# CESSProject/DeOSS

Hardware: AMD Instinct MI355X
Metric: device-resident GiB/s hashed to Merkle root; 1/2/4/8 MI355X scaling (higher is better)
Workload: dtype u32; 1 GPU; BASELINE configs[1]: 1 object of 8 GiB (8589934592 B) in 1 chunk-range shard(s) of 8 GiB, chunk 33554432 B (256 leaves); object_bytes=8589934592, chunk=33554432, leaves=256, parallelism=single GPU

## Files before the change

deoss_amd/csrc/merkle_kernels.hpp:

```cpp
#pragma once
#include "quad_ring.hpp"
#include "sha256_gfx950.hpp"

namespace dm {

constexpr int kBlock = 256;
constexpr int kLeafFuseMax = 8;
constexpr int kReduceTile = 512;

struct LeafArgs {
    const uint8_t* base;
    uint64_t pitch;
    uint64_t leaf_len;
    uint64_t last_len;
    const uint64_t* addrs;
    const uint64_t* lens;
    uint64_t nleaves;
    uint64_t byte_off;
    uint64_t byte_end;
    uint32_t* state;
    uint8_t* digests;
    uint8_t* level_out;
    uint32_t fuse_levels;
};
// ... 345 lines not shown
#pragma unroll
        for (int k = 0; k < 8; k++) o8[k] = res[threadIdx.x][k];
        const uint64_t o = (uint64_t)blockIdx.x * (kLatLeaves >> a.fuse_levels) + threadIdx.x;
        store_digest(a.level_out + 32 * o, o8);
    }
}

constexpr int kPairLeaves = 32;
constexpr int kPairFuseMax = 5;

__device__ __forceinline__ uint32_t dpp_swap_pairs(uint32_t v) {
    return (uint32_t)__builtin_amdgcn_update_dpp(0, (int)v, 0xB1, 0xF, 0xF, true);
}

#define DM_PAIR_ROUND(X4, X5, X6, X7, kw)                                              \
    do {                                                                               \
        const uint32_t s_ = xor3(__builtin_amdgcn_alignbit(X4, X4, sh1),               \
                                 __builtin_amdgcn_alignbit(X4, X4, sh2),               \
                                 __builtin_amdgcn_alignbit(X4, X4, sh3));              \
        const uint32_t x_ = __builtin_amdgcn_bitop3_b32(X4, X5, msk, 0x1e);            \
        const uint32_t f_ = __builtin_amdgcn_bitop3_b32(x_, X6, X5, 0xca);             \
        const uint32_t t_ = s_ + f_ + ((X7 & msk) + (kw));                             \
        const uint32_t y_ = lane_b ? X7 : t_;                                          \
        X7 = t_ + dpp_swap_pairs(y_);                                                  \
    } while (0)

__device__ __forceinline__ void pair_rounds_from_kw(uint32_t (&x)[4], const uint4 (*kw)[kLatLeaves], uint32_t lane,
                                                    uint32_t sh1, uint32_t sh2, uint32_t sh3, uint32_t msk,
                                                    bool lane_b) {
    uint32_t x4 = x[0], x5 = x[1], x6 = x[2], x7 = x[3];
    uint4 q = kw[0][lane];
#pragma unroll
    for (int g = 0; g < 16; g++) {
        uint4 nq = q;
        if (g + 1 < 16) nq = kw[g + 1][lane];
        DM_PAIR_ROUND(x4, x5, x6, x7, q.x);
        DM_PAIR_ROUND(x7, x4, x5, x6, q.y);
        DM_PAIR_ROUND(x6, x7, x4, x5, q.z);
        DM_PAIR_ROUND(x5, x6, x7, x4, q.w);
        q = nq;
    }
    x[0] += x4; x[1] += x5; x[2] += x6; x[3] += x7;
}

template <bool TABLE, bool ALIGNED>
__global__ __launch_bounds__(kLatThreads) void leaf_kernel_pair(LeafArgs a) {
    __shared__ uint4 ring[kLatRing][16][kLatLeaves];
    __shared__ uint32_t lds_a[kPairLeaves][8];
    __shared__ uint32_t lds_b[kPairLeaves / 2][8];
    const uint32_t lane = threadIdx.x & (kLatLeaves - 1);
    const bool producer = __builtin_amdgcn_readfirstlane(threadIdx.x) < kLatLeaves;
    const bool lane_b = (lane & 1) != 0;
    const uint32_t c = lane >> 1;
    const uint64_t first = (uint64_t)blockIdx.x * kPairLeaves;
    const uint64_t i = first + c;
    const LeafView v = leaf_view<TABLE>(a, i);
    const uint64_t NB = wave_max_u64(v.nb);
    if (producer) {
        Blk cur;
        if (v.nb > 0 && !lane_b) cur = load_block<ALIGNED>(v.p);
        for (uint64_t b = 0; b < NB; b++) {
            if (b < v.nb) {
                uint32_t w[16];
                block_words(cur, w);
                if (b + 1 < v.nb && !lane_b) cur = load_block<ALIGNED>(v.p + 64 * (b + 1));
                uint4 (*kw)[kLatLeaves] = ring[b % kLatRing];
#pragma unroll
                for (int q = 0; q < 16; q++) {
                    uint32_t u[4];
#pragma unroll
                    for (int j = 0; j < 4; j++) {
                        const int t = 4 * q + j;
                        uint32_t wt;
                        if (t < 16) {
                            wt = w[t];
                        } else {
                            wt = ssig1(w[(t - 2) & 15]) + w[(t - 7) & 15] + ssig0(w[(t - 15) & 15]) + w[t & 15];
                            w[t & 15] = wt;
                        }
                        u[j] = lane_b ? 0u : kSha256K[t] + wt;
                    }
                    kw[q][lane] = make_uint4(u[0], u[1], u[2], u[3]);
                }
            }
            __syncthreads();
        }
        __syncthreads();
    } else {
        const uint32_t sh1 = lane_b ? 2 : 6, sh2 = lane_b ? 13 : 11, sh3 = lane_b ? 22 : 25;
        const uint32_t msk = lane_b ? 0u : ~0u;
        uint32_t st0[8];
        if (v.active) load_or_init_state(a, i, st0);
        else init_state(st0);
        uint32_t x[4];
#pragma unroll
        for (int k = 0; k < 4; k++) x[k] = lane_b ? st0[k] : st0[4 + k];
        __syncthreads();
        for (uint64_t b = 0; b < NB; b++) {
            if (b < v.nb) pair_rounds_from_kw(x, ring[b % kLatRing], lane, sh1, sh2, sh3, msk, lane_b);
            __syncthreads();
        }
        uint32_t st[8];
#pragma unroll
        for (int k = 0; k < 4; k++) {
            const uint32_t other = dpp_swap_pairs(x[k]);
            st[k] = lane_b ? x[k] : other;
            st[4 + k] = lane_b ? other : x[k];
        }
        if (v.active && !lane_b) {
            leaf_epilogue<ALIGNED>(a, i, v, st);
#pragma unroll
            for (int k = 0; k < 8; k++) lds_a[c][k] = st[k];
        }
    }
    if (a.fuse_levels == 0) return;
    __syncthreads();
    const uint32_t cnt = (uint32_t)((a.nleaves - first) < kPairLeaves ? (a.nleaves - first) : kPairLeaves);
    uint32_t (*res)[8];
    const uint32_t out_cnt = lds_reduce(lds_a, lds_b, cnt, a.fuse_levels, &res);
    if (threadIdx.x < out_cnt) {
        uint32_t o8[8];
#pragma unroll
        for (int k = 0; k < 8; k++) o8[k] = res[threadIdx.x][k];
        const uint64_t o = (uint64_t)blockIdx.x * (kPairLeaves >> a.fuse_levels) + threadIdx.x;
        store_digest(a.level_out + 32 * o, o8);
    }
}

constexpr int kQuadLeaves = 8;
constexpr int kQuadBlocks = 8;
constexpr int kQuadFuseMax = 3;
constexpr int kQuadRow = kQuadLeaves;
constexpr size_t kQuadLdsBytes = sizeof(uint4) * kLatRing * 16 * kQuadBlocks * kQuadRow + 4 * 8 * kQuadLeaves +
                                 4 * 8 * (kQuadLeaves / 2);
static_assert(4 * kQuadLdsBytes <= (160u << 10), "four compact K1Q workgroups must fit a CU's LDS");

#define DM_QS_HEAD(X4, X5, X6)                                                                   \
    "v_alignbit_b32 %[r], %[" X4 "], %[" X4 "], %[sh]\n\t"                                      \
    "v_bitop3_b32 %[f], %[" X4 "], %[" X5 "], %[msk] bitop3:0x1e\n\t"                          \
    "v_bitop3_b32 %[f], %[f], %[" X6 "], %[" X5 "] bitop3:0xca\n\t"                             \
    "v_xor_b32_dpp %[s], %[r], %[r] quad_perm:[1,2,0,3] row_mask:0xf bank_mask:0xf\n\t"
#define DM_QS_SIGMA "v_xor_b32_dpp %[s], %[r], %[s] quad_perm:[2,0,1,3] row_mask:0xf bank_mask:0xf\n\t"
#define DM_QS_STEP_Q(X4, X5, X6, X7, H, HN, VN, QP)                                             \
    DM_QS_HEAD(X4, X5, X6)                                                                       \
    "v_sub_u32_dpp %[" X6 "], %[" VN "], %[" X6 "] quad_perm:" QP " row_mask:0xf bank_mask:0x3\n\t" \
    DM_QS_SIGMA                                                                                  \
    "v_sub_u32_dpp %[" HN "], %[" X4 "], %[" X6 "] row_ror:8 row_mask:0xf bank_mask:0xf\n\t"    \
    "v_add3_u32 %[" X7 "], %[s], %[f], %[" H "]\n\t"
#define DM_QS_STEP(X4, X5, X6, X7, H, HN, VN) DM_QS_STEP_Q(X4, X5, X6, X7, H, HN, VN, "[0,1,2,3]")
#define DM_QS_STEP_A(X4, X5, X6, X7, H, HN)                                                     \
    DM_QS_HEAD(X4, X5, X6)                                                                       \
    DM_QS_SIGMA                                                                                  \
    "v_sub_u32_dpp %[" HN "], %[" X4 "], %[" X6 "] row_ror:8 row_mask:0xf bank_mask:0xf\n\t"    \
    "v_add3_u32 %[" X7 "], %[s], %[f], %[" H "]\n\t"
#define DM_QS_STEP_END(X4, X5, X6, X7, H)                                                       \
    DM_QS_HEAD(X4, X5, X6)                                                                       \
    DM_QS_SIGMA                                                                                  \
    "v_add3_u32 %[" X7 "], %[s], %[f], %[" H "]\n\t"
#define DM_QS_STEPS4V(V0, V1, V2, V3)                                                          \
    DM_QS_STEP("a", "b", "c", "d", "h", "g", V0) DM_QS_STEP("d", "a", "b", "c", "g", "h", V1)   \
    DM_QS_STEP("c", "d", "a", "b", "h", "g", V2) DM_QS_STEP("b", "c", "d", "a", "g", "h", V3)
#define DM_QS_ALIGN_MIS ".p2align 3\n\t.if %[mis]\n\ts_nop 0\n\t.endif\n\t"
#define DM_QS_PROLOGUE(V) DM_QS_PROLOGUE_AT(V, DM_QS_ALIGN_MIS, "[0,1,2,3]")
#define DM_QS_PROLOGUE_AT(V, ALIGN, QP)                                                           \
    "s_nop 1\n\t" ALIGN                                                                          \
    "v_sub_u32_dpp %[d], %[" V "], %[d] quad_perm:" QP " row_mask:0xf bank_mask:0x3\n\t"         \
    "v_sub_u32_dpp %[h], %[b], %[d] row_ror:8 row_mask:0xf bank_mask:0xf\n\t"
#define DM_QS_RESTORE_A(P, X) "v_mov_b32_dpp %[" P "], %[" X "] quad_perm:[0,1,2,3] row_mask:0xf bank_mask:0xc\n\t"
#define DM_QS_GROUP0(V0, V1, V2, V3)                                                             \
    DM_QS_STEP("a", "b", "c", "d", "h", "g", V0) DM_QS_RESTORE_A("d", "x3")                      \
    DM_QS_STEP("d", "a", "b", "c", "g", "h", V1) DM_QS_RESTORE_A("c", "x2")                      \
    DM_QS_STEP("c", "d", "a", "b", "h", "g", V2) DM_QS_STEP("b", "c", "d", "a", "g", "h", V3)
#define DM_QS_FF(X, P, BANKS) "v_add_u32_dpp %[" X "], %[" P "], %[" X "] quad_perm:[0,1,2,3] row_mask:0xf bank_mask:" BANKS "\n\t"
#define DM_QS_TAIL(V0, V1, V2)                                                                   \
    DM_QS_STEP("a", "b", "c", "d", "h", "g", V0) DM_QS_STEP("d", "a", "b", "c", "g", "h", V1)   \
    DM_QS_STEP("c", "d", "a", "b", "h", "g", V2) DM_QS_STEP_A("b", "c", "d", "a", "g", "h")      \
    DM_QS_FF("x3", "d", "0x3") DM_QS_FF("x2", "c", "0x3") DM_QS_FF("x1", "b", "0x3")             \
    DM_QS_FF("x0", "a", "0x3")                                                                   \
    DM_QS_STEP_A("a", "b", "c", "d", "h", "g") DM_QS_STEP_END("d", "a", "b", "c", "g")           \
    DM_QS_FF("x0", "a", "0xc") DM_QS_FF("x1", "b", "0xc") DM_QS_FF("x3", "d", "0xc")             \
    DM_QS_FF("x2", "c", "0xc")
#define DM_QS_STEPS4Q(V0, Q0, V1, Q1, V2, Q2, V3, Q3)                                          \
    DM_QS_STEP_Q("a", "b", "c", "d", "h", "g", V0, Q0) DM_QS_STEP_Q("d", "a", "b", "c", "g", "h", V1, Q1) \
    DM_QS_STEP_Q("c", "d", "a", "b", "h", "g", V2, Q2) DM_QS_STEP_Q("b", "c", "d", "a", "g", "h", V3, Q3)
#define DM_QS_GROUP0Q(V0, Q0, V1, Q1, V2, Q2, V3, Q3)                                          \
    DM_QS_STEP_Q("a", "b", "c", "d", "h", "g", V0, Q0) DM_QS_RESTORE_A("d", "x3")              \
    DM_QS_STEP_Q("d", "a", "b", "c", "g", "h", V1, Q1) DM_QS_RESTORE_A("c", "x2")              \
    DM_QS_STEP_Q("c", "d", "a", "b", "h", "g", V2, Q2) DM_QS_STEP_Q("b", "c", "d", "a", "g", "h", V3, Q3)
#define DM_QS_TAILQ(V0, Q0, V1, Q1, V2, Q2)                                                     \
    DM_QS_STEP_Q("a", "b", "c", "d", "h", "g", V0, Q0) DM_QS_STEP_Q("d", "a", "b", "c", "g", "h", V1, Q1) \
    DM_QS_STEP_Q("c", "d", "a", "b", "h", "g", V2, Q2) DM_QS_STEP_A("b", "c", "d", "a", "g", "h") \
    DM_QS_FF("x3", "d", "0x3") DM_QS_FF("x2", "c", "0x3") DM_QS_FF("x1", "b", "0x3")             \
    DM_QS_FF("x0", "a", "0x3")                                                                   \
    DM_QS_STEP_A("a", "b", "c", "d", "h", "g") DM_QS_STEP_END("d", "a", "b", "c", "g")           \
    DM_QS_FF("x0", "a", "0xc") DM_QS_FF("x1", "b", "0xc") DM_QS_FF("x3", "d", "0xc")             \
    DM_QS_FF("x2", "c", "0xc")
#define DM_QS_OUT                                                                                \
    : [a] "+v"(p0), [b] "+v"(p1), [c] "+v"(p2), [d] "+v"(p3), [h] "+v"(h), [g] "+v"(g),           \
      [x0] "+v"(x[0]), [x1] "+v"(x[1]), [x2] "+v"(x[2]), [x3] "+v"(x[3]), [r] "=&v"(r_),          \
      [f] "=&v"(f_), [s] "=&v"(s_)
#define DM_QS_OPS DM_QS_OUT : [mis] "i"(MIS ? 1 : 0), [sh] "v"(sh.x), [msk] "v"(msk), [v0] "v"(v0), [v1] "v"(v1), [v2] "v"(v2), [v3] "v"(v3)

template <bool MIS, class KW>
__device__ __forceinline__ void quad_block_skewed(uint32_t (&x)[4], KW kw, uint3 sh, uint32_t msk) {
    uint32_t p0 = x[0], p1 = x[1], p2 = x[2], p3 = x[3], h = 0, g = 0, r_, f_, s_;
    uint4 q = kw(0), nq = kw(1);
    {
        const uint32_t v0 = q.x, v1 = 0, v2 = 0, v3 = 0;
        asm volatile(DM_QS_PROLOGUE("v0") DM_QS_OPS);
    }
#pragma unroll
    for (int grp = 0; grp < 16; grp++) {
        const uint4 nnq = grp + 2 < 16 ? kw(grp + 2) : nq;
        const uint32_t v0 = q.y, v1 = q.z, v2 = q.w, v3 = nq.x;
        if (grp == 0) {
            asm volatile(DM_QS_ALIGN_MIS DM_QS_GROUP0("v0", "v1", "v2", "v3") DM_QS_OPS);
        } else if (grp < 15) {
            asm volatile(DM_QS_ALIGN_MIS DM_QS_STEPS4V("v0", "v1", "v2", "v3") DM_QS_OPS);
        } else {
            asm volatile(DM_QS_ALIGN_MIS DM_QS_TAIL("v0", "v1", "v2") DM_QS_OPS);
        }
        q = nq;
        nq = nnq;
    }
}

constexpr int kLgkmWait0 = 0xC07F;

#define DM_QS_HNB(HN, A, B, BANKS) "v_sub_u32_dpp %[" HN "], %[" A "], %[" B "] row_ror:8 row_mask:0xf bank_mask:" BANKS "\n\t"
#define DM_QS_ADDB(D, A, B, BANKS) "v_add_u32_dpp %[" D "], %[" A "], %[" B "] quad_perm:[0,1,2,3] row_mask:0xf bank_mask:" BANKS "\n\t"
#define DM_QS_MOVB(D, S, BANKS) "v_mov_b32_dpp %[" D "], %[" S "] quad_perm:[0,1,2,3] row_mask:0xf bank_mask:" BANKS "\n\t"
#define DM_QS_KWN(X6, S, N) "v_sub_u32_dpp %[" X6 "], %[" N "], %[" S "] quad_perm:[0,0,0,0] row_mask:0xf bank_mask:0x3\n\t"
#define DM_QS_ADD3(X7, H) "v_add3_u32 %[" X7 "], %[s], %[f], %[" H "]\n\t"
#define DM_QS_LINKQ(V0, Q0, V1, Q1, V2, Q2, N0, N1, N2)                                          \
    DM_QS_STEP_Q("a", "b", "c", "d", "h", "g", V0, Q0) DM_QS_STEP_Q("d", "a", "b", "c", "g", "h", V1, Q1) \
    DM_QS_STEP_Q("c", "d", "a", "b", "h", "g", V2, Q2)                                           \
    DM_QS_ADDB("x1", "x1", "b", "0xc") DM_QS_ADDB("x3", "x3", "d", "0x3")                        \
                                            \
    DM_QS_HEAD("b", "c", "d") DM_QS_KWN("d", "x3", N0) DM_QS_SIGMA                               \
    DM_QS_HNB("h", "x1", "d", "0x3") DM_QS_HNB("h", "b", "d", "0xc") DM_QS_ADD3("a", "g")        \
    DM_QS_ADDB("b", "x1", "b", "0x3") DM_QS_ADDB("c", "x2", "c", "0x3")                          \
    DM_QS_HNB("g", "a", "c", "0xc") DM_QS_ADDB("x0", "x0", "a", "0xc")                           \
    DM_QS_ADDB("a", "a", "x0", "0x3") DM_QS_MOVB("x2", "c", "0x3")                               \
                                                            \
    DM_QS_HEAD("a", "b", "c") DM_QS_KWN("c", "c", N1) DM_QS_SIGMA                                \
    DM_QS_HNB("g", "x0", "c", "0x3") DM_QS_ADD3("d", "h")                                        \
    DM_QS_ADDB("x3", "x3", "d", "0xc") DM_QS_MOVB("x1", "b", "0x3") DM_QS_MOVB("x0", "a", "0x3") \
                                           \
    DM_QS_HEAD("d", "a", "b") DM_QS_KWN("b", "b", N2) DM_QS_SIGMA                                \
    DM_QS_HNB("h", "x3", "b", "0x3") DM_QS_HNB("h", "d", "x1", "0xc") DM_QS_ADD3("c", "g")       \
    DM_QS_ADDB("x2", "x2", "c", "0xc") DM_QS_MOVB("a", "x0", "0xc") DM_QS_MOVB("d", "x3", "0xc") \
    DM_QS_MOVB("c", "x2", "0xc")
#define DM_QS_BODYQ                                                                              \
    DM_QS_STEPS4Q("q01", "[1,1,1,1]", "q02", "[1,1,1,1]", "q03", "[1,1,1,1]", "q00", "[2,2,2,2]") \
    DM_QS_STEPS4Q("q01", "[2,2,2,2]", "q02", "[2,2,2,2]", "q03", "[2,2,2,2]", "q00", "[3,3,3,3]") \
    DM_QS_STEPS4Q("q01", "[3,3,3,3]", "q02", "[3,3,3,3]", "q03", "[3,3,3,3]", "q10", "[0,0,0,0]") \
    DM_QS_STEPS4Q("q11", "[0,0,0,0]", "q12", "[0,0,0,0]", "q13", "[0,0,0,0]", "q10", "[1,1,1,1]") \
    DM_QS_STEPS4Q("q11", "[1,1,1,1]", "q12", "[1,1,1,1]", "q13", "[1,1,1,1]", "q10", "[2,2,2,2]") \
    DM_QS_STEPS4Q("q11", "[2,2,2,2]", "q12", "[2,2,2,2]", "q13", "[2,2,2,2]", "q10", "[3,3,3,3]") \
    DM_QS_STEPS4Q("q11", "[3,3,3,3]", "q12", "[3,3,3,3]", "q13", "[3,3,3,3]", "q20", "[0,0,0,0]") \
    DM_QS_STEPS4Q("q21", "[0,0,0,0]", "q22", "[0,0,0,0]", "q23", "[0,0,0,0]", "q20", "[1,1,1,1]") \
    DM_QS_STEPS4Q("q21", "[1,1,1,1]", "q22", "[1,1,1,1]", "q23", "[1,1,1,1]", "q20", "[2,2,2,2]") \
    DM_QS_STEPS4Q("q21", "[2,2,2,2]", "q22", "[2,2,2,2]", "q23", "[2,2,2,2]", "q20", "[3,3,3,3]") \
    DM_QS_STEPS4Q("q21", "[3,3,3,3]", "q22", "[3,3,3,3]", "q23", "[3,3,3,3]", "q30", "[0,0,0,0]") \
    DM_QS_STEPS4Q("q31", "[0,0,0,0]", "q32", "[0,0,0,0]", "q33", "[0,0,0,0]", "q30", "[1,1,1,1]") \
    DM_QS_STEPS4Q("q31", "[1,1,1,1]", "q32", "[1,1,1,1]", "q33", "[1,1,1,1]", "q30", "[2,2,2,2]") \
    DM_QS_STEPS4Q("q31", "[2,2,2,2]", "q32", "[2,2,2,2]", "q33", "[2,2,2,2]", "q30", "[3,3,3,3]")
#define DM_QS_FILLQ                                                                              \
    DM_QS_PROLOGUE_AT("q00", DM_QS_ALIGN_MIS, "[0,0,0,0]")                                       \
    DM_QS_GROUP0Q("q01", "[0,0,0,0]", "q02", "[0,0,0,0]", "q03", "[0,0,0,0]", "q00", "[1,1,1,1]")
#define DM_QS_CONTQ                                                                              \
    DM_QS_ALIGN_MIS                                                                              \
    DM_QS_STEP_Q("c", "d", "a", "b", "h", "g", "q03", "[0,0,0,0]") DM_QS_STEP_Q("b", "c", "d", "a", "g", "h", "q00", "[1,1,1,1]")
#define DM_QS_ENDLINKQ DM_QS_LINKQ("q31", "[3,3,3,3]", "q32", "[3,3,3,3]", "q33", "[3,3,3,3]", "n0", "n1", "n2")
#define DM_QS_ENDTAILQ DM_QS_TAILQ("q31", "[3,3,3,3]", "q32", "[3,3,3,3]", "q33", "[3,3,3,3]")
#define DM_QS_STATE [a] "+v"(P[0]), [b] "+v"(P[1]), [c] "+v"(P[2]), [d] "+v"(P[3]),              \
                    [x0] "+v"(x[0]), [x1] "+v"(x[1]), [x2] "+v"(x[2]), [x3] "+v"(x[3]),           \
                    [r] "=&v"(r_), [f] "=&v"(f_), [s] "=&v"(s_)
#define DM_QS_KIN [mis] "i"(MIS ? 1 : 0), [sh] "v"(sh.x), [msk] "v"(msk),                        \
                  [q00] "v"(K[0].x), [q01] "v"(K[0].y), [q02] "v"(K[0].z), [q03] "v"(K[0].w),     \
                  [q10] "v"(K[1].x), [q11] "v"(K[1].y), [q12] "v"(K[1].z), [q13] "v"(K[1].w),     \
                  [q20] "v"(K[2].x), [q21] "v"(K[2].y), [q22] "v"(K[2].z), [q23] "v"(K[2].w),     \
                  [q30] "v"(K[3].x), [q31] "v"(K[3].y), [q32] "v"(K[3].z), [q33] "v"(K[3].w)

template <bool MIS, int K8>
__device__ __forceinline__ void quad_block_regs(uint32_t (&x)[4], uint32_t (&P)[4], uint32_t& h, uint32_t& g,
                                                const uint4 (&K)[4], const uint4& N, uint3 sh, uint32_t msk) {
    uint32_t r_, f_, s_;
    if constexpr (K8 == 0) {
        asm volatile(DM_QS_FILLQ DM_QS_BODYQ DM_QS_ENDLINKQ
                     : DM_QS_STATE, [h] "=&v"(h), [g] "=&v"(g)
                     : DM_QS_KIN, [n0] "v"(N.x), [n1] "v"(N.y), [n2] "v"(N.z));
    } else if constexpr (K8 < kQuadBlocks - 1) {
        asm volatile(DM_QS_CONTQ DM_QS_BODYQ DM_QS_ENDLINKQ
                     : DM_QS_STATE, [h] "+v"(h), [g] "+v"(g)
                     : DM_QS_KIN, [n0] "v"(N.x), [n1] "v"(N.y), [n2] "v"(N.z));
    } else {
        asm volatile(DM_QS_CONTQ DM_QS_BODYQ DM_QS_ENDTAILQ
                     : DM_QS_STATE, [h] "+v"(h), [g] "+v"(g)
                     : DM_QS_KIN);
    }
}

template <int G, int ROW, bool MIS, int K8 = 0>
__device__ __forceinline__ void quad_stage_blocks(uint32_t (&x)[4], uint32_t (&P)[4], uint32_t& h, uint32_t& g,
                                                  uint4 (&S)[3][4], const uint4* kw, uint3 sh, uint32_t msk) {
    __builtin_amdgcn_s_waitcnt(kLgkmWait0);
    if constexpr (K8 + 2 < kQuadBlocks) {
#pragma unroll
        for (int t = 0; t < 4; t++) S[(K8 + 2) % 3][t] = kw[(K8 + 2) * ROW + 4 * t * G];
    }
    quad_block_regs<MIS, K8>(x, P, h, g, S[K8 % 3], S[(K8 + 1) % 3][0], sh, msk);
    if constexpr (K8 + 1 < kQuadBlocks) quad_stage_blocks<G, ROW, MIS, K8 + 1>(x, P, h, g, S, kw, sh, msk);
}
template <int G, int ROW, bool MIS>
__device__ __forceinline__ void quad_stage_regs(uint32_t (&x)[4], const uint4* kw, uint3 sh, uint32_t msk) {
    uint4 S[3][4];
    uint32_t P[4] = {x[0], x[1], x[2], x[3]}, h, g;
#pragma unroll
    for (int k = 0; k < 2; k++) {
#pragma unroll
        for (int t = 0; t < 4; t++) S[k][t] = kw[k * ROW + 4 * t * G];
    }
    quad_stage_blocks<G, ROW, MIS>(x, P, h, g, S, kw, sh, msk);
}

constexpr int kQuadWideRing = quad_ring::kWideDepth;
constexpr int kQuadSets = quad_ring::kSets;
template <int G, int ROW, int K8, bool FILL, bool TAIL, bool LOAD>
__device__ __forceinline__ void quad_xstage_block(uint32_t (&x)[4], uint32_t (&P)[4], uint32_t& h, uint32_t& g,
                                                  uint4 (&S)[kQuadSets][4], const uint4* src, uint3 sh, uint32_t msk) {
    static_assert((LOAD || !quad_ring::block_prefetches(K8, true)) && (!TAIL || !quad_ring::block_links(K8, true)) &&
                      !(FILL && TAIL) && quad_ring::prefetch_of(K8).block == (K8 + quad_ring::kAhead) % kQuadBlocks,
                  "only the last stage of a run skips a load or drains: quad_ring.hpp");
    __builtin_amdgcn_s_waitcnt(kLgkmWait0);
    if constexpr (LOAD) {
        constexpr quad_ring::BlockRef pf = quad_ring::prefetch_of(K8);
#pragma unroll
        for (int t = 0; t < 4; t++) S[quad_ring::set_of(K8 + quad_ring::kAhead)][t] = src[pf.block * ROW + 4 * t * G];
    }
    quad_block_regs<false, FILL ? 0 : TAIL ? kQuadBlocks - 1 : 1>(x, P, h, g, S[quad_ring::set_of(K8)],
                                                                 S[quad_ring::set_of(K8 + 1)][0], sh, msk);
}
template <int G, int ROW>
__device__ __forceinline__ uint32_t quad_run_xstage(uint32_t (&x)[4], const uint4* colp, uint32_t slot, uint64_t n,
                                                    uint3 sh, uint32_t msk) {
    uint4 S[kQuadSets][4];
    uint32_t P[4] = {x[0], x[1], x[2], x[3]}, h, g;
    const uint4* cur = colp + slot * 16 * G;
#pragma unroll
    for (int k = 0; k < quad_ring::kAhead; k++) {
#pragma unroll
        for (int t = 0; t < 4; t++) S[k][t] = cur[k * ROW + 4 * t * G];
    }
    quad_xstage_block<G, ROW, 0, true, false, true>(x, P, h, g, S, cur, sh, msk);
    for (uint64_t s = 1; s < n; s++) {
        slot = quad_ring::next_slot(slot, kQuadWideRing);
        const uint4* nxt = colp + slot * 16 * G;
        quad_xstage_block<G, ROW, 1, false, false, true>(x, P, h, g, S, cur, sh, msk);
        quad_xstage_block<G, ROW, 2, false, false, true>(x, P, h, g, S, cur, sh, msk);
        quad_xstage_block<G, ROW, 3, false, false, true>(x, P, h, g, S, cur, sh, msk);
        quad_xstage_block<G, ROW, 4, false, false, true>(x, P, h, g, S, cur, sh, msk);
        quad_xstage_block<G, ROW, 5, false, false, true>(x, P, h, g, S, cur, sh, msk);
        quad_xstage_block<G, ROW, 6, false, false, true>(x, P, h, g, S, nxt, sh, msk);
        quad_xstage_block<G, ROW, 7, false, false, true>(x, P, h, g, S, nxt, sh, msk);
        __syncthreads();
        quad_xstage_block<G, ROW, 0, false, false, true>(x, P, h, g, S, nxt, sh, msk);
        cur = nxt;
    }
    quad_xstage_block<G, ROW, 1, false, false, true>(x, P, h, g, S, cur, sh, msk);
    quad_xstage_block<G, ROW, 2, false, false, true>(x, P, h, g, S, cur, sh, msk);
    quad_xstage_block<G, ROW, 3, false, false, true>(x, P, h, g, S, cur, sh, msk);
    quad_xstage_block<G, ROW, 4, false, false, true>(x, P, h, g, S, cur, sh, msk);
    quad_xstage_block<G, ROW, 5, false, false, true>(x, P, h, g, S, cur, sh, msk);
    quad_xstage_block<G, ROW, 6, false, false, false>(x, P, h, g, S, cur, sh, msk);
    quad_xstage_block<G, ROW, 7, false, true, false>(x, P, h, g, S, cur, sh, msk);
    __syncthreads();
    return quad_ring::next_slot(slot, kQuadWideRing);
}

template <bool ALIGNED, int G>
__device__ __forceinline__ void quad_produce_block(const LeafView& v, Blk& cur, uint64_t b, uint4* kw) {
    if (b >= v.nb) return;
    uint32_t w[16];
    block_words(cur, w);
    if (b + kQuadBlocks < v.nb) cur = load_block<ALIGNED>(v.p + 64 * (b + kQuadBlocks));
#pragma unroll
    for (int q = 0; q < 16; q++) {
        uint32_t u[4];
#pragma unroll
        for (int k = 0; k < 4; k++) {
            const int t = 4 * q + k;
            uint32_t wt;
            if (t < 16) {
                wt = w[t];
            } else {
                wt = ssig1(w[(t - 2) & 15]) + w[(t - 7) & 15] + ssig0(w[(t - 15) & 15]) + w[t & 15];
                w[t & 15] = wt;
            }
            u[k] = 0u - (kSha256K[t] + wt);
        }
        kw[q * G] = make_uint4(u[0], u[1], u[2], u[3]);
    }
}

template <bool TABLE, bool ALIGNED, bool COMPACT>
__global__ __launch_bounds__(kLatThreads) void leaf_kernel_quad(LeafArgs a) {
    constexpr int ROW = COMPACT ? kQuadRow : kQuadLeaves;
    constexpr int G = kQuadBlocks * ROW;
    constexpr int DEPTH = COMPACT ? kLatRing : kQuadWideRing;
    __shared__ uint4 ring[COMPACT ? 1 : 2][kLatRing][16][G];
    __shared__ uint32_t lds_a[kQuadLeaves][8];
    __shared__ uint32_t lds_b[kQuadLeaves / 2][8];
    static_assert(DEPTH * sizeof(ring[0][0]) <= sizeof(ring), "the ring's stages must fit its LDS");
    static_assert(COMPACT || (3 * sizeof(ring) > (160u << 10) && sizeof(ring) <= (64u << 10) &&
                              2 * (sizeof(ring) + sizeof(lds_a) + sizeof(lds_b)) <= (160u << 10)),
                  "the wide K1Q must stay at exactly two workgroups per CU (160 KiB of LDS)");
    const uint32_t lane = threadIdx.x & 63;
    const bool producer = __builtin_amdgcn_readfirstlane(threadIdx.x) < 64;
    const uint32_t c = lane >> 3;
    const uint32_t j = lane & 7;
    const uint64_t first = (uint64_t)blockIdx.x * kQuadLeaves;
    const uint64_t i = first + c;
    const LeafView v = leaf_view<TABLE>(a, i);
    const uint64_t NB = wave_max_u64(v.nb);
    const uint64_t NI = (NB + kQuadBlocks - 1) / kQuadBlocks;
    if (producer) {
        Blk cur;
        if (j < v.nb) cur = load_block<ALIGNED>(v.p + 64 * j);
        if constexpr (!COMPACT) {
            uint4* const kw0 = &ring[0][0][0][j * ROW + c];
            uint32_t slot = 0;
            for (uint64_t s = 0; s < quad_ring::stages_before_first_barrier(DEPTH); s++) {
                if (s < NI) quad_produce_block<ALIGNED, G>(v, cur, s * kQuadBlocks + j, kw0 + slot * 16 * G);
                slot = quad_ring::next_slot(slot, DEPTH);
            }
            __syncthreads();
            for (uint64_t it = 0; it < NI; it++) {
                const uint64_t s = quad_ring::stage_written_after_barrier(it, DEPTH);
                if (s < NI) quad_produce_block<ALIGNED, G>(v, cur, s * kQuadBlocks + j, kw0 + slot * 16 * G);
                slot = quad_ring::next_slot(slot, DEPTH);
                __syncthreads();
            }
        } else {
            for (uint64_t it = 0; it < NI; it++) {
                const uint64_t b = it * kQuadBlocks + j;
                if (b < v.nb) {
                    uint32_t w[16];
                    block_words(cur, w);
                    if (b + kQuadBlocks < v.nb) cur = load_block<ALIGNED>(v.p + 64 * (b + kQuadBlocks));
                    uint4* kw = &ring[0][it % kLatRing][0][j * ROW + c];
#pragma unroll
                    for (int q = 0; q < 16; q++) {
                        uint32_t u[4];
#pragma unroll
                        for (int k = 0; k < 4; k++) {
                            const int t = 4 * q + k;
                            uint32_t wt;
                            if (t < 16) {
                                wt = w[t];
                            } else {
                                wt = ssig1(w[(t - 2) & 15]) + w[(t - 7) & 15] + ssig0(w[(t - 15) & 15]) + w[t & 15];
                                w[t & 15] = wt;
                            }
                            u[k] = 0u - (kSha256K[t] + wt);
                        }
                        kw[q * G] = make_uint4(u[0], u[1], u[2], u[3]);
                    }
                }
                __syncthreads();
            }
            __syncthreads();
        }
    } else {
        __builtin_amdgcn_s_setprio(1);
        const uint32_t cq = 2 * (lane >> 4) + ((lane >> 2) & 1);
        const bool role_a = (lane >> 3) & 1;
        const uint32_t p = lane & 3;
        const uint64_t iq = first + cq;
        const LeafView vq = leaf_view<TABLE>(a, iq);
        const uint3 sh = make_uint3(role_a ? (p == 0 ? 2 : p == 1 ? 13 : 22) : (p == 0 ? 6 : p == 1 ? 11 : 25), 0, 0);
        const uint32_t msk = role_a ? 0u : ~0u;
        uint32_t st0[8];
        if (vq.active) load_or_init_state(a, iq, st0);
        else init_state(st0);
        uint32_t x[4];
#pragma unroll
        for (int k = 0; k < 4; k++) x[k] = role_a ? st0[(k + 2) & 3] : st0[4 + k];
        const uint4* col = &ring[0][0][0][cq];
        __syncthreads();
        uint32_t xf[4];
#pragma unroll
        for (int k = 0; k < 4; k++) xf[k] = x[k];
        const uint64_t NS = uniform_u64(NI);
        uint32_t wslot = 0;
        for (uint64_t it = 0; it < NS;) {
            const bool running = COMPACT ? vq.active && vq.nb > it * kQuadBlocks
                                         : quad_ring::leaf_running(vq.active, vq.nb, it);
            const uint64_t end = uniform_u64(wave_min_u64(COMPACT ? (running ? vq.nb / kQuadBlocks : NS)
                                                                  : quad_ring::leaf_run_end(running, vq.nb, NS)));
            if constexpr (COMPACT) {
                for (; it < end; it++) {
                    quad_stage_regs<G, ROW, COMPACT>(x, col + (it % kLatRing) * 16 * G + p * G, sh, msk);
                    __syncthreads();
                }
            } else if (it < end) {
                wslot = quad_run_xstage<G, ROW>(x, col + p * G, wslot, end - it, sh, msk);
                it = end;
            }
            if (running) {
#pragma unroll
                for (int k = 0; k < 4; k++) xf[k] = x[k];
            }
            if (it == NS) break;
            if (!__any(COMPACT ? vq.active && vq.nb > it * kQuadBlocks && vq.nb < (it + 1) * kQuadBlocks
                               : quad_ring::leaf_ends_inside(vq.active, vq.nb, it)))
                continue;
            const uint4* kw = col + (COMPACT ? (uint32_t)(it % kLatRing) : wslot) * 16 * G;
            const uint64_t b0 = it * kQuadBlocks;
            for (uint32_t k = 0; k < kQuadBlocks; k++) {
                const uint4* kb = kw + k * ROW;
                if (b0 + k < vq.nb)
                    quad_block_skewed<COMPACT>(x, [kb](int g) { return kb[g * G]; }, sh, msk);
            }
            if (vq.nb > b0) {
#pragma unroll
                for (int k = 0; k < 4; k++) xf[k] = x[k];
            }
            __syncthreads();
            it++;
            wslot = quad_ring::next_slot(wslot, DEPTH);
        }
        uint32_t st[8];
#pragma unroll
        for (int k = 0; k < 4; k++) {
            st[k] = __shfl(xf[(k + 2) & 3], (int)(lane + 8), 64);
            st[4 + k] = xf[k];
        }
        if (vq.active && !role_a && p == 0) {
            leaf_epilogue<ALIGNED>(a, iq, vq, st);
#pragma unroll
            for (int k = 0; k < 8; k++) lds_a[cq][k] = st[k];
        }
    }
    if (a.fuse_levels == 0) return;
    __syncthreads();
    const uint32_t cnt = (uint32_t)((a.nleaves - first) < kQuadLeaves ? (a.nleaves - first) : kQuadLeaves);
    uint32_t (*res)[8];
    const uint32_t out_cnt = lds_reduce(lds_a, lds_b, cnt, a.fuse_levels, &res);
    if (threadIdx.x < out_cnt) {
        uint32_t o8[8];
#pragma unroll
        for (int k = 0; k < 8; k++) o8[k] = res[threadIdx.x][k];
        const uint64_t o = (uint64_t)blockIdx.x * (kQuadLeaves >> a.fuse_levels) + threadIdx.x;
        store_digest(a.level_out + 32 * o, o8);
    }
}

__global__ __launch_bounds__(kLatThreads) void quad_shape_primer(int x) {
    extern __shared__ uint4 dyn[];
    if (x == 12345) dyn[threadIdx.x] = make_uint4(1, 1, 1, 1);
}

__global__ __launch_bounds__(kBlock) void reduce_kernel(const uint8_t* in, uint64_t m, uint32_t levels,
                                                         uint8_t* out) {
    __shared__ uint32_t lds_a[kBlock][8];
    __shared__ uint32_t lds_b[kBlock / 2][8];
    const uint64_t base = (uint64_t)blockIdx.x * kReduceTile;
    const uint32_t cnt = (uint32_t)((m - base) < kReduceTile ? (m - base) : kReduceTile);
    const uint32_t t = threadIdx.x;
    const uint32_t next = (cnt + 1) >> 1;
    if (t < next) {
        uint32_t L[8], R[8], o[8];
        const uint32_t ri = (2 * t + 1 < cnt) ? 2 * t + 1 : cnt - 1;
        load_digest(in + 32 * (base + 2 * t), L);
        load_digest(in + 32 * (base + ri), R);
        node_hash(L, R, o);
#pragma unroll
        for (int k = 0; k < 8; k++) lds_a[t][k] = o[k];
    }
    __syncthreads();
    uint32_t (*res)[8];
    const uint32_t out_cnt = lds_reduce(lds_a, lds_b, next, levels - 1, &res);
    if (t < out_cnt) {
        uint32_t v[8];
#pragma unroll
        for (int k = 0; k < 8; k++) v[k] = res[t][k];
        store_digest(out + 32 * ((uint64_t)blockIdx.x * (kReduceTile >> levels) + t), v);
    }
}

__global__ __launch_bounds__(kBlock) void batch_root_kernel(const uint8_t* leaves, const uint64_t* leaf_first,
                                                             const uint32_t* obj_ids, uint8_t* roots) {
    __shared__ uint32_t lds_a[kBlock][8];
    __shared__ uint32_t lds_b[kBlock / 2][8];
    const uint32_t o = obj_ids[blockIdx.x];
    const uint64_t base = leaf_first[o];
    const uint32_t cnt = (uint32_t)(leaf_first[o + 1] - base);
    const uint32_t t = threadIdx.x;
    const uint32_t next = (cnt + 1) >> 1;
    if (t < next) {
        uint32_t L[8], R[8], h[8];
        const uint32_t ri = (2 * t + 1 < cnt) ? 2 * t + 1 : cnt - 1;
        load_digest(leaves + 32 * (base + 2 * t), L);
        load_digest(leaves + 32 * (base + ri), R);
        node_hash(L, R, h);
#pragma unroll
        for (int k = 0; k < 8; k++) lds_a[t][k] = h[k];
    }
    __syncthreads();
    uint32_t levels = 0;
    for (uint32_t c = next; c > 1; c = (c + 1) >> 1) levels++;
    uint32_t (*res)[8];
    lds_reduce(lds_a, lds_b, next, levels, &res);
    if (t == 0) {
        uint32_t v[8];
#pragma unroll
        for (int k = 0; k < 8; k++) v[k] = res[0][k];
        store_digest(roots + 32 * (uint64_t)o, v);
    }
}

__device__ __forceinline__ uint64_t splitmix64(uint64_t z) {
    z += 0x9e3779b97f4a7c15ULL;
    z = (z ^ (z >> 30)) * 0xbf58476d1ce4e5b9ULL;
    z = (z ^ (z >> 27)) * 0x94d049bb133111ebULL;
    return z ^ (z >> 31);
}

__global__ __launch_bounds__(kBlock) void fill_splitmix_kernel(uint64_t* dst, uint64_t word0, uint64_t nwords,
                                                                uint64_t seed) {
    const uint64_t stride = (uint64_t)gridDim.x * kBlock * 2;
    for (uint64_t j = ((uint64_t)blockIdx.x * kBlock + threadIdx.x) * 2; j < nwords; j += stride) {
        if (j + 1 < nwords) {
            ulonglong2 v = make_ulonglong2(splitmix64(seed ^ (word0 + j)), splitmix64(seed ^ (word0 + j + 1)));
            *reinterpret_cast<ulonglong2*>(dst + j) = v;
        } else {
            dst[j] = splitmix64(seed ^ (word0 + j));
        }
    }
}

constexpr int kProbeLoads = 16;
__global__ __launch_bounds__(kBlock) void read_probe_kernel(const uint8_t* p, uint64_t n16, uint64_t* out) {
    const u32x4_t* g = reinterpret_cast<const u32x4_t*>(p);
    const uint64_t per = (n16 + gridDim.x - 1) / gridDim.x;
    const uint64_t lo = (uint64_t)blockIdx.x * per, hi = lo + per < n16 ? lo + per : n16;
    u32x4_t acc[kProbeLoads];
#pragma unroll
    for (int u = 0; u < kProbeLoads; u++) acc[u] = u32x4_t{0u, 0u, 0u, 0u};
    uint64_t i = lo + threadIdx.x;
    for (; i + (kProbeLoads - 1) * kBlock < hi; i += kProbeLoads * kBlock) {
        u32x4_t x[kProbeLoads];
#pragma unroll
        for (int u = 0; u < kProbeLoads; u++) x[u] = __builtin_nontemporal_load(g + i + u * kBlock);
#pragma unroll
        for (int u = 0; u < kProbeLoads; u++) acc[u] ^= x[u];
    }
    for (; i < hi; i += kBlock) acc[0] ^= g[i];
#pragma unroll
    for (int u = 1; u < kProbeLoads; u++) acc[0] ^= acc[u];
    uint64_t v = (((uint64_t)acc[0].y << 32) | acc[0].x) ^ (((uint64_t)acc[0].w << 32) | acc[0].z);
    for (int m = 32; m >= 1; m >>= 1) v ^= __shfl_xor(v, m, 64);
    __shared__ uint64_t part[kBlock / 64];
    if ((threadIdx.x & 63) == 0) part[threadIdx.x >> 6] = v;
    __syncthreads();
    if (threadIdx.x == 0) {
        uint64_t t = 0;
        for (int w = 0; w < kBlock / 64; w++) t ^= part[w];
        atomicXor(reinterpret_cast<unsigned long long*>(out), (unsigned long long)t);
    }
}

}
```

Before: 16.93 GiB/s.

## Ping-pong SHA-256 working state across register banks in the wide quad-stage path

Adds a wide inline-asm SHA-256 block variant that alternates the working state between two register banks (a..d and x0..x3) on even and odd blocks. It keeps five extra link values live across blocks so the feed-forward addition and next-block setup can interleave with the final rounds instead of serializing. The aim is to cut move and dependency stalls at block boundaries in the ring-buffered column hashing loop. In exchange it raises VGPR pressure, which could reduce occupancy, and the hand-written register dataflow is fragile to get right.

```diff
diff --git a/deoss_amd/csrc/merkle_kernels.hpp b/deoss_amd/csrc/merkle_kernels.hpp
--- a/deoss_amd/csrc/merkle_kernels.hpp
+++ b/deoss_amd/csrc/merkle_kernels.hpp
@@ -671,6 +671,94 @@
     }
 }
 
+#define DM_QS_WSTEPS4(W0, W1, W2, W3, V0, Q0, V1, Q1, V2, Q2, V3, Q3)                            \
+    DM_QS_STEP_Q(W0, W1, W2, W3, "h", "g", V0, Q0) DM_QS_STEP_Q(W3, W0, W1, W2, "g", "h", V1, Q1) \
+    DM_QS_STEP_Q(W2, W3, W0, W1, "h", "g", V2, Q2) DM_QS_STEP_Q(W1, W2, W3, W0, "g", "h", V3, Q3)
+#define DM_QS_WLINK(W0, W1, W2, W3, C0, C1, C2, C3, Y2, Y3, Z2, Z3)                              \
+    DM_QS_STEP_Q(W0, W1, W2, W3, "h", "g", "q31", "[3,3,3,3]")                                   \
+    DM_QS_STEP_Q(W3, W0, W1, W2, "g", "h", "q32", "[3,3,3,3]")                                   \
+    DM_QS_STEP_Q(W2, W3, W0, W1, "h", "g", "q33", "[3,3,3,3]")                                   \
+    DM_QS_ADDB("w", "w", W1, "0xc")                                                              \
+                                            \
+    DM_QS_HEAD(W1, W2, W3) DM_QS_ADDB(W3, C3, W3, "0x3") DM_QS_KWN("t", W3, "n0") DM_QS_SIGMA    \
+    DM_QS_HNB("h", "w", "t", "0x3") DM_QS_HNB("h", W1, W3, "0xc") DM_QS_ADD3(W0, "g")            \
+    DM_QS_ADDB(W1, C1, W1, "0x3") DM_QS_ADDB(W2, C2, W2, "0x3")                                  \
+    DM_QS_HNB("g", W0, W2, "0xc") DM_QS_ADDB(W0, C0, W0, "0x3")                                  \
+                                \
+    DM_QS_HEAD(W0, W1, W2) DM_QS_KWN("u", W2, "n1") DM_QS_SIGMA DM_QS_ADD3(Y3, "h")              \
+                                           \
+    DM_QS_HEAD(Y3, W0, W1) DM_QS_ADDB(W0, C0, W0, "0xc") DM_QS_ADDB(Y3, Z3, Y3, "0xc")           \
+    DM_QS_KWN("t", W1, "n2") DM_QS_SIGMA                                                         \
+    DM_QS_HNB("g", W0, "u", "0x3") DM_QS_HNB("h", Y3, "t", "0x3") DM_QS_HNB("h", Y3, "w", "0xc") \
+    DM_QS_ADD3(Y2, "g") DM_QS_ADDB(Y2, Z2, Y2, "0xc")
+#define DM_QS_WCONT(W0, W1, W2, W3, C0, Z2, Z3)                                                  \
+    DM_QS_ALIGN_MIS                                                                              \
+    DM_QS_HEAD(Z2, Z3, C0) DM_QS_KWN("t", C0, "q03") DM_QS_SIGMA                                 \
+    DM_QS_HNB("g", Z2, "t", "0x3") DM_QS_HNB("g", Z2, C0, "0xc") DM_QS_ADD3(W1, "h")             \
+    DM_QS_STEP_Q(W1, Z2, Z3, W0, "g", "h", "q00", "[1,1,1,1]")                                   \
+    DM_QS_STEP_Q(W0, W1, Z2, W3, "h", "g", "q01", "[1,1,1,1]")                                   \
+    DM_QS_STEP_Q(W3, W0, W1, W2, "g", "h", "q02", "[1,1,1,1]")                                   \
+    DM_QS_STEP_Q(W2, W3, W0, W1, "h", "g", "q03", "[1,1,1,1]")                                   \
+    DM_QS_STEP_Q(W1, W2, W3, W0, "g", "h", "q00", "[2,2,2,2]")
+#define DM_QS_WREST(W0, W1, W2, W3)                                                              \
+    DM_QS_WSTEPS4(W0, W1, W2, W3, "q01", "[2,2,2,2]", "q02", "[2,2,2,2]", "q03", "[2,2,2,2]", "q00", "[3,3,3,3]") \
+    DM_QS_WSTEPS4(W0, W1, W2, W3, "q01", "[3,3,3,3]", "q02", "[3,3,3,3]", "q03", "[3,3,3,3]", "q10", "[0,0,0,0]") \
+    DM_QS_WSTEPS4(W0, W1, W2, W3, "q11", "[0,0,0,0]", "q12", "[0,0,0,0]", "q13", "[0,0,0,0]", "q10", "[1,1,1,1]") \
+    DM_QS_WSTEPS4(W0, W1, W2, W3, "q11", "[1,1,1,1]", "q12", "[1,1,1,1]", "q13", "[1,1,1,1]", "q10", "[2,2,2,2]") \
+    DM_QS_WSTEPS4(W0, W1, W2, W3, "q11", "[2,2,2,2]", "q12", "[2,2,2,2]", "q13", "[2,2,2,2]", "q10", "[3,3,3,3]") \
+    DM_QS_WSTEPS4(W0, W1, W2, W3, "q11", "[3,3,3,3]", "q12", "[3,3,3,3]", "q13", "[3,3,3,3]", "q20", "[0,0,0,0]") \
+    DM_QS_WSTEPS4(W0, W1, W2, W3, "q21", "[0,0,0,0]", "q22", "[0,0,0,0]", "q23", "[0,0,0,0]", "q20", "[1,1,1,1]") \
+    DM_QS_WSTEPS4(W0, W1, W2, W3, "q21", "[1,1,1,1]", "q22", "[1,1,1,1]", "q23", "[1,1,1,1]", "q20", "[2,2,2,2]") \
+    DM_QS_WSTEPS4(W0, W1, W2, W3, "q21", "[2,2,2,2]", "q22", "[2,2,2,2]", "q23", "[2,2,2,2]", "q20", "[3,3,3,3]") \
+    DM_QS_WSTEPS4(W0, W1, W2, W3, "q21", "[3,3,3,3]", "q22", "[3,3,3,3]", "q23", "[3,3,3,3]", "q30", "[0,0,0,0]") \
+    DM_QS_WSTEPS4(W0, W1, W2, W3, "q31", "[0,0,0,0]", "q32", "[0,0,0,0]", "q33", "[0,0,0,0]", "q30", "[1,1,1,1]") \
+    DM_QS_WSTEPS4(W0, W1, W2, W3, "q31", "[1,1,1,1]", "q32", "[1,1,1,1]", "q33", "[1,1,1,1]", "q30", "[2,2,2,2]") \
+    DM_QS_WSTEPS4(W0, W1, W2, W3, "q31", "[2,2,2,2]", "q32", "[2,2,2,2]", "q33", "[2,2,2,2]", "q30", "[3,3,3,3]")
+#define DM_QS_WTAIL(W0, W1, W2, W3, C0, C1, C2, C3, Y2, Y3, Z2, Z3)                              \
+    DM_QS_STEP_Q(W0, W1, W2, W3, "h", "g", "q31", "[3,3,3,3]")                                   \
+    DM_QS_STEP_Q(W3, W0, W1, W2, "g", "h", "q32", "[3,3,3,3]")                                   \
+    DM_QS_STEP_Q(W2, W3, W0, W1, "h", "g", "q33", "[3,3,3,3]")                                   \
+    DM_QS_STEP_A(W1, W2, W3, W0, "g", "h") DM_QS_STEP_A(W0, W1, W2, Y3, "h", "g")                \
+    DM_QS_STEP_END(Y3, W0, W1, Y2, "g")                                                          \
+    DM_QS_ADDB(W0, C0, W0, "0xf") DM_QS_ADDB(W1, C1, W1, "0x3") DM_QS_ADDB(W2, C2, W2, "0x3")    \
+    DM_QS_ADDB(W3, C3, W3, "0x3") DM_QS_ADDB(W1, "w", W1, "0xc") DM_QS_ADDB(W2, Z2, Y2, "0xc")   \
+    DM_QS_ADDB(W3, Z3, Y3, "0xc")
+#define DM_QS_WLINK_EVEN DM_QS_WLINK("a", "b", "c", "d", "x0", "x1", "x2", "x3", "y2", "y3", "z2", "z3")
+#define DM_QS_WLINK_ODD DM_QS_WLINK("x0", "x1", "x2", "x3", "a", "b", "c", "d", "z2", "z3", "y2", "y3")
+#define DM_QS_WCONT_EVEN DM_QS_WCONT("a", "b", "c", "d", "x0", "z2", "z3")
+#define DM_QS_WCONT_ODD DM_QS_WCONT("x0", "x1", "x2", "x3", "a", "y2", "y3")
+#define DM_QS_WREST_EVEN DM_QS_WREST("a", "b", "c", "d")
+#define DM_QS_WREST_ODD DM_QS_WREST("x0", "x1", "x2", "x3")
+#define DM_QS_WTAIL_ODD DM_QS_WTAIL("x0", "x1", "x2", "x3", "a", "b", "c", "d", "z2", "z3", "y2", "y3")
+#define DM_QS_WSTATE DM_QS_STATE, [h] "+v"(h), [g] "+v"(g), [w] "+v"(L[0]), [y2] "+v"(L[1]),   \
+                     [y3] "+v"(L[2]), [z2] "+v"(L[3]), [z3] "+v"(L[4]), [t] "=&v"(t_), [u] "=&v"(u_)
+
+template <int K8, bool FILL, bool TAIL>
+__device__ __forceinline__ void quad_block_wide(uint32_t (&x)[4], uint32_t (&P)[4], uint32_t& h, uint32_t& g,
+                                                uint32_t (&L)[5], const uint4 (&K)[4], const uint4& N, uint3 sh,
+                                                uint32_t msk) {
+    static_assert(!(FILL && (K8 & 1)) && !(TAIL && !(K8 & 1)), "a run fills on an even block and drains on an odd one");
+    constexpr bool MIS = false;
+    uint32_t r_, f_, s_, t_, u_;
+    if constexpr (FILL) {
+        asm volatile(DM_QS_FILLQ DM_QS_BODYQ DM_QS_WLINK_EVEN
+                     : DM_QS_WSTATE
+                     : DM_QS_KIN, [n0] "v"(N.x), [n1] "v"(N.y), [n2] "v"(N.z));
+    } else if constexpr (TAIL) {
+        asm volatile(DM_QS_WCONT_ODD DM_QS_WREST_ODD DM_QS_WTAIL_ODD
+                     : DM_QS_WSTATE
+                     : DM_QS_KIN);
+    } else if constexpr (K8 & 1) {
+        asm volatile(DM_QS_WCONT_ODD DM_QS_WREST_ODD DM_QS_WLINK_ODD
+                     : DM_QS_WSTATE
+                     : DM_QS_KIN, [n0] "v"(N.x), [n1] "v"(N.y), [n2] "v"(N.z));
+    } else {
+        asm volatile(DM_QS_WCONT_EVEN DM_QS_WREST_EVEN DM_QS_WLINK_EVEN
+                     : DM_QS_WSTATE
+                     : DM_QS_KIN, [n0] "v"(N.x), [n1] "v"(N.y), [n2] "v"(N.z));
+    }
+}
+
 template <int G, int ROW, bool MIS, int K8 = 0>
 __device__ __forceinline__ void quad_stage_blocks(uint32_t (&x)[4], uint32_t (&P)[4], uint32_t& h, uint32_t& g,
                                                   uint4 (&S)[3][4], const uint4* kw, uint3 sh, uint32_t msk) {
@@ -698,7 +786,8 @@
 constexpr int kQuadSets = quad_ring::kSets;
 template <int G, int ROW, int K8, bool FILL, bool TAIL, bool LOAD>
 __device__ __forceinline__ void quad_xstage_block(uint32_t (&x)[4], uint32_t (&P)[4], uint32_t& h, uint32_t& g,
-                                                  uint4 (&S)[kQuadSets][4], const uint4* src, uint3 sh, uint32_t msk) {
+                                                  uint32_t (&L)[5], uint4 (&S)[kQuadSets][4], const uint4* src,
+                                                  uint3 sh, uint32_t msk) {
     static_assert((LOAD || !quad_ring::block_prefetches(K8, true)) && (!TAIL || !quad_ring::block_links(K8, true)) &&
                       !(FILL && TAIL) && quad_ring::prefetch_of(K8).block == (K8 + quad_ring::kAhead) % kQuadBlocks,
                   "only the last stage of a run skips a load or drains: quad_ring.hpp");
@@ -708,42 +797,42 @@
 #pragma unroll
         for (int t = 0; t < 4; t++) S[quad_ring::set_of(K8 + quad_ring::kAhead)][t] = src[pf.block * ROW + 4 * t * G];
     }
-    quad_block_regs<false, FILL ? 0 : TAIL ? kQuadBlocks - 1 : 1>(x, P, h, g, S[quad_ring::set_of(K8)],
-                                                                 S[quad_ring::set_of(K8 + 1)][0], sh, msk);
+    quad_block_wide<K8, FILL, TAIL>(x, P, h, g, L, S[quad_ring::set_of(K8)], S[quad_ring::set_of(K8 + 1)][0], sh, msk);
 }
 template <int G, int ROW>
 __device__ __forceinline__ uint32_t quad_run_xstage(uint32_t (&x)[4], const uint4* colp, uint32_t slot, uint64_t n,
                                                     uint3 sh, uint32_t msk) {
     uint4 S[kQuadSets][4];
-    uint32_t P[4] = {x[0], x[1], x[2], x[3]}, h, g;
+    uint32_t P[4] = {x[0], x[1], x[2], x[3]}, h = 0, g = 0;
+    uint32_t L[5] = {x[1], 0, 0, x[2], x[3]};
     const uint4* cur = colp + slot * 16 * G;
 #pragma unroll
     for (int k = 0; k < quad_ring::kAhead; k++) {
 #pragma unroll
         for (int t = 0; t < 4; t++) S[k][t] = cur[k * ROW + 4 * t * G];
     }
-    quad_xstage_block<G, ROW, 0, true, false, true>(x, P, h, g, S, cur, sh, msk);
+    quad_xstage_block<G, ROW, 0, true, false, true>(x, P, h, g, L, S, cur, sh, msk);
     for (uint64_t s = 1; s < n; s++) {
         slot = quad_ring::next_slot(slot, kQuadWideRing);
         const uint4* nxt = colp + slot * 16 * G;
-        quad_xstage_block<G, ROW, 1, false, false, true>(x, P, h, g, S, cur, sh, msk);
-        quad_xstage_block<G, ROW, 2, false, false, true>(x, P, h, g, S, cur, sh, msk);
-        quad_xstage_block<G, ROW, 3, false, false, true>(x, P, h, g, S, cur, sh, msk);
-        quad_xstage_block<G, ROW, 4, false, false, true>(x, P, h, g, S, cur, sh, msk);
-        quad_xstage_block<G, ROW, 5, false, false, true>(x, P, h, g, S, cur, sh, msk);
-        quad_xstage_block<G, ROW, 6, false, false, true>(x, P, h, g, S, nxt, sh, msk);
-        quad_xstage_block<G, ROW, 7, false, false, true>(x, P, h, g, S, nxt, sh, msk);
+        quad_xstage_block<G, ROW, 1, false, false, true>(x, P, h, g, L, S, cur, sh, msk);
+        quad_xstage_block<G, ROW, 2, false, false, true>(x, P, h, g, L, S, cur, sh, msk);
+        quad_xstage_block<G, ROW, 3, false, false, true>(x, P, h, g, L, S, cur, sh, msk);
+        quad_xstage_block<G, ROW, 4, false, false, true>(x, P, h, g, L, S, cur, sh, msk);
+        quad_xstage_block<G, ROW, 5, false, false, true>(x, P, h, g, L, S, cur, sh, msk);
+        quad_xstage_block<G, ROW, 6, false, false, true>(x, P, h, g, L, S, nxt, sh, msk);
+        quad_xstage_block<G, ROW, 7, false, false, true>(x, P, h, g, L, S, nxt, sh, msk);
         __syncthreads();
-        quad_xstage_block<G, ROW, 0, false, false, true>(x, P, h, g, S, nxt, sh, msk);
+        quad_xstage_block<G, ROW, 0, false, false, true>(x, P, h, g, L, S, nxt, sh, msk);
         cur = nxt;
     }
-    quad_xstage_block<G, ROW, 1, false, false, true>(x, P, h, g, S, cur, sh, msk);
-    quad_xstage_block<G, ROW, 2, false, false, true>(x, P, h, g, S, cur, sh, msk);
-    quad_xstage_block<G, ROW, 3, false, false, true>(x, P, h, g, S, cur, sh, msk);
-    quad_xstage_block<G, ROW, 4, false, false, true>(x, P, h, g, S, cur, sh, msk);
-    quad_xstage_block<G, ROW, 5, false, false, true>(x, P, h, g, S, cur, sh, msk);
-    quad_xstage_block<G, ROW, 6, false, false, false>(x, P, h, g, S, cur, sh, msk);
-    quad_xstage_block<G, ROW, 7, false, true, false>(x, P, h, g, S, cur, sh, msk);
+    quad_xstage_block<G, ROW, 1, false, false, true>(x, P, h, g, L, S, cur, sh, msk);
+    quad_xstage_block<G, ROW, 2, false, false, true>(x, P, h, g, L, S, cur, sh, msk);
+    quad_xstage_block<G, ROW, 3, false, false, true>(x, P, h, g, L, S, cur, sh, msk);
+    quad_xstage_block<G, ROW, 4, false, false, true>(x, P, h, g, L, S, cur, sh, msk);
+    quad_xstage_block<G, ROW, 5, false, false, true>(x, P, h, g, L, S, cur, sh, msk);
+    quad_xstage_block<G, ROW, 6, false, false, false>(x, P, h, g, L, S, cur, sh, msk);
+    quad_xstage_block<G, ROW, 7, false, true, false>(x, P, h, g, L, S, cur, sh, msk);
     __syncthreads();
     return quad_ring::next_slot(slot, kQuadWideRing);
 }
```

Measured after the change: 17.04 GiB/s, median of 6. About the same (+0.7%).
